# parthjaggi/flow

Measured on AMD Instinct MI355X. Metric: env-steps/sec, higher is better.
Workload: dtype mixed

## Files before the change

flow_amd/csrc/flowsim_pair.h:

```cpp
#pragma once
#include "flowsim_kernels.h"

namespace fs {

typedef float f2 __attribute__((ext_vector_type(2)));
typedef unsigned u2v __attribute__((__vector_size__(8)));

enum : int { DPP_ROW_NEWBCAST0 = 0x150, DPP_ROW_NEWBCAST8 = 0x158 };

__device__ __forceinline__ f2 fma2(f2 a, f2 b, f2 c) { return __builtin_elementwise_fma(a, b, c); }
__device__ __forceinline__ f2 splat(float a) { return f2{a, a}; }

__device__ __forceinline__ f2 pk_mul(f2 a, f2 b) { return a * b; }
__device__ __forceinline__ f2 pk_add(f2 a, f2 b) { return a + b; }
__device__ __forceinline__ f2 pk_sub(f2 a, f2 b) { return a - b; }
__device__ __forceinline__ f2 pk_fma(f2 a, f2 b, f2 c) { return fma2(a, b, c); }
__device__ __forceinline__ f2 pk_fnma(f2 a, f2 b, f2 c) { return fma2(-a, b, c); }
__device__ __forceinline__ float nonneg_else(float x, float y) {
  const unsigned a = __builtin_bit_cast(unsigned, x), b = __builtin_bit_cast(unsigned, y);
  return __builtin_bit_cast(float, min(a, b));
}

template <int ROW>
__device__ __forceinline__ float next_a(float v, bool last, int lane) {
// ... 113 lines not shown
#include "flowsim_pair_step_a_sm.inc"
#undef FS_PAIR_A_NAME
#undef FS_PAIR_A_NZ
#undef FS_PAIR_A_NZ_PARAM
#define FS_PAIR_A_NAME pair_step_asm_a_sm_nz
#define FS_PAIR_A_NZ 1
#define FS_PAIR_A_NZ_PARAM , f2 nz
#include "flowsim_pair_step_a_sm.inc"
#undef FS_PAIR_A_NAME
#undef FS_PAIR_A_NZ
#undef FS_PAIR_A_NZ_PARAM
__device__ __forceinline__ void pair_step_asm_b(f2& V, f2& X, f2& H, f2& DVL, f2& OV, unsigned& crash_bits, float& sq,
                                                const PairConsts& c) {
  asm volatile(
      "v_sub_f32_e32 v118, v112, v113\n"
      "v_sub_f32_e32 v132, v115, v114\n"
      "v_subrev_f32_dpp v119, v112, v113 row_shl:1 row_mask:0xf bank_mask:0xf bound_ctrl:1\n"
      "v_subrev_f32_dpp v134, v112, v113 row_newbcast:0 row_mask:0xf bank_mask:0xf\n"
      "v_sub_f32_dpp v133, v114, v115 row_shl:1 row_mask:0xf bank_mask:0xf bound_ctrl:1\n"
      "v_sub_f32_dpp v135, v114, v115 row_newbcast:0 row_mask:0xf bank_mask:0xf\n"
      "v_cndmask_b32_e64 v119, v119, v134, %[last]\n"
      "v_cndmask_b32_e64 v133, v133, v135, %[last]\n"
      "v_pk_add_f32 v[126:127], v[132:133], %[L2]\n"
      "v_min_u32_e32 v132, v132, v126\n"
      "v_min_u32_e32 v133, v133, v127\n"
      "v_pk_add_f32 v[116:117], v[132:133], %[lenlead] neg_lo:[0,1] neg_hi:[0,1]\n"
      "v_pk_add_f32 v[126:127], v[116:117], %[gap2] neg_lo:[0,1] neg_hi:[0,1]\n"
      "v_min_f32_e32 v126, v126, v127\n"
      "v_alignbit_b32 %[cb], %[cb], v126, 31\n"
      "v_pk_fma_f32 v[124:125], v[112:113], %[vmask], %[tvm]\n"
      "v_pk_mul_f32 v[124:125], v[124:125], v[124:125]\n"
      "v_add_f32_e32 %[sq], v124, v125\n"
      "v_cvt_f64_f32_e32 v[130:131], v112\n"
      "v_cvt_f64_f32_e32 v[132:133], v113\n"
      "v_mul_f64 v[134:135], v[130:131], %[rcms]\n"
      "v_mul_f64 v[136:137], v[132:133], %[rcms]\n"
      "v_fma_f64 v[130:131], -v[134:135], %[ms], v[130:131]\n"
      "v_fma_f64 v[132:133], -v[136:137], %[ms], v[132:133]\n"
      "v_fma_f64 v[134:135], v[130:131], %[rcms], v[134:135]\n"
      "v_fma_f64 v[136:137], v[132:133], %[rcms], v[136:137]\n"
      "v_cvt_f32_f64_e32 v128, v[134:135]\n"
      "v_cvt_f32_f64_e32 v129, v[136:137]\n"
      : "+{v[112:113]}"(V), "+{v[114:115]}"(X), "+{v[116:117]}"(H), "+{v[118:119]}"(DVL), "={v[128:129]}"(OV),
        [cb] "+v"(crash_bits), [sq] "=&v"(sq)
      : [L2] "v"(c.L2), [lenlead] "v"(c.len_lead), [gap2] "v"(c.gap2), [vmask] "v"(c.vmask), [tvm] "v"(c.tvm),
        [ms] "v"(c.ms64), [rcms] "v"(c.rc_ms64), [last] "s"(c.last_mask)
      : "v124", "v125", "v126", "v127", "v130", "v131", "v132", "v133", "v134", "v135", "v136", "v137");
}

struct MixedConsts {
  f2 p0, p1, p2, p5, rc_v0, tsab, rc_ab, one, gap2, vmask, tvm;
  float c1e3;
  double dt, ramp, L, rc_L, rc_ms, len_b, len_next, zero;
  unsigned long long last_mask;
};
__device__ __forceinline__ void mixed_step_asm_a(f2& V32, double& XA, double& XB, double& VA, double& VB, f2& H, f2& DVL,
                                                 f2& OV, const MixedConsts& c) {
  unsigned long long sa, sb;
  asm volatile(
      "v_cmp_nlt_f32_e64 %[sa], |v140|, %[c1e3]\n"
      "v_cmp_nlt_f32_e64 %[sb], |v141|, %[c1e3]\n"
      "v_pk_mul_f32 v[124:125], v[112:113], v[142:143]\n"
      "v_pk_mul_f32 v[126:127], v[124:125], %[rcab]\n"
      "v_pk_fma_f32 v[130:131], v[126:127], %[tsab], v[124:125] neg_lo:[1,0,0] neg_hi:[1,0,0]\n"
      "v_pk_fma_f32 v[126:127], v[130:131], %[rcab], v[126:127]\n"
      "v_cndmask_b32_e64 v120, %[c1e3], v140, %[sa]\n"
      "v_cndmask_b32_e64 v121, %[c1e3], v141, %[sb]\n"
      "v_pk_mul_f32 v[124:125], v[112:113], %[rcv0]\n"
      "v_rcp_f32_e32 v122, v120\n"
      "v_rcp_f32_e32 v123, v121\n"
      "v_pk_fma_f32 v[130:131], v[124:125], %[p0], v[112:113] neg_lo:[1,0,0] neg_hi:[1,0,0]\n"
      "v_pk_fma_f32 v[124:125], v[130:131], %[rcv0], v[124:125]\n"
      "v_pk_mul_f32 v[130:131], v[112:113], %[p1]\n"
      "v_pk_add_f32 v[130:131], v[130:131], v[126:127]\n"
      "v_pk_fma_f32 v[126:127], v[120:121], v[122:123], %[one] neg_lo:[1,0,0] neg_hi:[1,0,0]\n"
      "v_max_f32_e32 v130, 0, v130\n"
      "v_max_f32_e32 v131, 0, v131\n"
      "v_pk_fma_f32 v[122:123], v[126:127], v[122:123], v[122:123]\n"
      "v_pk_add_f32 v[130:131], %[p5], v[130:131]\n"
      "v_pk_mul_f32 v[124:125], v[124:125], v[124:125]\n"
      "v_pk_mul_f32 v[126:127], v[130:131], v[122:123]\n"
      "v_pk_mul_f32 v[124:125], v[124:125], v[124:125]\n"
      "v_pk_fma_f32 v[132:133], v[120:121], v[126:127], v[130:131] neg_lo:[1,0,0] neg_hi:[1,0,0]\n"
      "v_pk_add_f32 v[124:125], %[one], v[124:125] neg_lo:[0,1] neg_hi:[0,1]\n"
      "v_pk_fma_f32 v[126:127], v[132:133], v[122:123], v[126:127]\n"
      "v_pk_fma_f32 v[132:133], v[120:121], v[126:127], v[130:131] neg_lo:[1,0,0] neg_hi:[1,0,0]\n"
      "v_pk_fma_f32 v[126:127], v[132:133], v[122:123], v[126:127]\n"
      "v_pk_mul_f32 v[126:127], v[126:127], v[126:127]\n"
      "v_pk_add_f32 v[124:125], v[124:125], v[126:127] neg_lo:[0,1] neg_hi:[0,1]\n"
      "v_pk_mul_f32 v[124:125], %[p2], v[124:125]\n"
      "v_cvt_f64_f32_e32 v[130:131], v124\n"
      "v_cvt_f64_f32_e32 v[132:133], v125\n"
      "v_mul_f64 v[130:131], v[130:131], %[dt]\n"
      "v_mul_f64 v[132:133], v[132:133], %[dt]\n"
      "v_add_f64 v[130:131], v[118:119], v[130:131]\n"
      "v_add_f64 v[132:133], v[138:139], v[132:133]\n"
      "v_max_f64 v[130:131], v[130:131], %[zero]\n"
      "v_max_f64 v[132:133], v[132:133], %[zero]\n"
      "v_add_f64 v[130:131], v[130:131], -v[118:119]\n"
      "v_add_f64 v[132:133], v[132:133], -v[138:139]\n"
      "v_mul_f64 v[130:131], v[130:131], %[ramp]\n"
      "v_mul_f64 v[132:133], v[132:133], %[ramp]\n"
      "v_add_f64 v[118:119], v[118:119], v[130:131]\n"
      "v_add_f64 v[138:139], v[138:139], v[132:133]\n"
      "v_mul_f64 v[130:131], v[118:119], %[dt]\n"
      "v_mul_f64 v[132:133], v[138:139], %[dt]\n"
      "v_add_f64 v[130:131], v[114:115], v[130:131]\n"
      "v_add_f64 v[132:133], v[116:117], v[132:133]\n"
      "v_add_f64 v[134:135], v[130:131], -%[L]\n"
      "v_add_f64 v[136:137], v[132:133], -%[L]\n"
      "v_cvt_f32_f64_e32 v112, v[118:119]\n"
      "v_cvt_f32_f64_e32 v113, v[138:139]\n"
      "v_cmp_gt_i32_e64 %[sa], 0, v135\n"
      "v_cmp_gt_i32_e64 %[sb], 0, v137\n"
      "v_mul_f64 v[120:121], v[118:119], %[rcms]\n"
      "v_mul_f64 v[122:123], v[138:139], %[rcms]\n"
      "v_cndmask_b32_e64 v114, v134, v130, %[sa]\n"
      "v_cndmask_b32_e64 v115, v135, v131, %[sa]\n"
      "v_cndmask_b32_e64 v116, v136, v132, %[sb]\n"
      "v_cndmask_b32_e64 v117, v137, v133, %[sb]\n"
      "v_cvt_f32_f64_e32 v128, v[120:121]\n"
      "v_cvt_f32_f64_e32 v129, v[122:123]\n"
      : "+{v[112:113]}"(V32), "+{v[114:115]}"(XA), "+{v[116:117]}"(XB), "+{v[118:119]}"(VA), "+{v[138:139]}"(VB),
        "+{v[140:141]}"(H), "+{v[142:143]}"(DVL), "={v[128:129]}"(OV), [sa] "=&s"(sa), [sb] "=&s"(sb)
      : [c1e3] "v"(c.c1e3), [rcab] "v"(c.rc_ab), [tsab] "v"(c.tsab), [rcv0] "v"(c.rc_v0), [p0] "v"(c.p0),
        [p1] "v"(c.p1), [p2] "v"(c.p2), [p5] "v"(c.p5), [one] "v"(c.one), [dt] "v"(c.dt), [ramp] "v"(c.ramp),
        [L] "v"(c.L), [rcms] "v"(c.rc_ms), [zero] "v"(c.zero)
      : "v120", "v121", "v122", "v123", "v124", "v125", "v126", "v127", "v130", "v131", "v132", "v133", "v134",
        "v135", "v136", "v137");
}
struct MixedSumoConsts { double fl0a, fl0b, adta, adtb, ddta, ddtb; };
__device__ __forceinline__ void mixed_step_asm_a_sm(f2& V32, double& XA, double& XB, double& VA, double& VB, f2& H,
                                                    f2& DVL, f2& OV, const MixedConsts& c, const SumoPair& m,
                                                    const MixedSumoConsts& d) {
  unsigned long long sa, sb;
  asm volatile(
      "v_cmp_nlt_f32_e64 %[sa], |v140|, %[c1e3]\n"
      "v_cmp_nlt_f32_e64 %[sb], |v141|, %[c1e3]\n"
      "v_pk_mul_f32 v[124:125], v[112:113], v[142:143]\n"
      "v_pk_mul_f32 v[126:127], v[124:125], %[rcab]\n"
      "v_pk_mul_f32 v[150:151], v[124:125], %[rcts]\n"
      "v_pk_fma_f32 v[130:131], v[126:127], %[tsab], v[124:125] neg_lo:[1,0,0] neg_hi:[1,0,0]\n"
      "v_pk_fma_f32 v[152:153], v[150:151], %[ts], v[124:125] neg_lo:[1,0,0] neg_hi:[1,0,0]\n"
      "v_pk_fma_f32 v[126:127], v[130:131], %[rcab], v[126:127]\n"
      "v_pk_fma_f32 v[150:151], v[152:153], %[rcts], v[150:151]\n"
      "v_cndmask_b32_e64 v120, %[c1e3], v140, %[sa]\n"
      "v_cndmask_b32_e64 v121, %[c1e3], v141, %[sb]\n"
      "v_max_f32_e32 v146, v140, %[c1e3]\n"
      "v_max_f32_e32 v147, v141, %[c1e3]\n"
      "v_pk_mul_f32 v[124:125], v[112:113], %[rcv0]\n"
      "v_rcp_f32_e32 v122, v120\n"
      "v_rcp_f32_e32 v123, v121\n"
      "v_rcp_f32_e32 v148, v146\n"
      "v_rcp_f32_e32 v149, v147\n"
      "v_pk_fma_f32 v[130:131], v[124:125], %[p0], v[112:113] neg_lo:[1,0,0] neg_hi:[1,0,0]\n"
      "v_pk_mul_f32 v[154:155], v[112:113], %[rcsm]\n"
      "v_pk_fma_f32 v[124:125], v[130:131], %[rcv0], v[124:125]\n"
      "v_pk_fma_f32 v[152:153], v[154:155], %[smax], v[112:113] neg_lo:[1,0,0] neg_hi:[1,0,0]\n"
      "v_pk_mul_f32 v[130:131], v[112:113], %[p1]\n"
      "v_pk_fma_f32 v[154:155], v[152:153], %[rcsm], v[154:155]\n"
      "v_pk_add_f32 v[130:131], v[130:131], v[126:127]\n"
      "v_pk_mul_f32 v[152:153], v[112:113], %[tau]\n"
      "v_pk_fma_f32 v[126:127], v[120:121], v[122:123], %[one] neg_lo:[1,0,0] neg_hi:[1,0,0]\n"
      "v_pk_add_f32 v[150:151], v[152:153], v[150:151]\n"
      "v_pk_fma_f32 v[152:153], v[146:147], v[148:149], %[one] neg_lo:[1,0,0] neg_hi:[1,0,0]\n"
      "v_max_f32_e32 v130, 0, v130\n"
      "v_max_f32_e32 v131, 0, v131\n"
      "v_max_f32_e32 v150, 0, v150\n"
      "v_max_f32_e32 v151, 0, v151\n"
      "v_pk_fma_f32 v[122:123], v[126:127], v[122:123], v[122:123]\n"
      "v_pk_fma_f32 v[148:149], v[152:153], v[148:149], v[148:149]\n"
      "v_pk_add_f32 v[130:131], %[p5], v[130:131]\n"
      "v_pk_add_f32 v[150:151], %[mgap], v[150:151]\n"
      "v_pk_mul_f32 v[124:125], v[124:125], v[124:125]\n"
      "v_pk_mul_f32 v[154:155], v[154:155], v[154:155]\n"
      "v_pk_mul_f32 v[126:127], v[130:131], v[122:123]\n"
      "v_pk_mul_f32 v[152:153], v[150:151], v[148:149]\n"
      "v_pk_mul_f32 v[124:125], v[124:125], v[124:125]\n"
      "v_pk_mul_f32 v[154:155], v[154:155], v[154:155]\n"
      "v_pk_fma_f32 v[132:133], v[120:121], v[126:127], v[130:131] neg_lo:[1,0,0] neg_hi:[1,0,0]\n"
      "v_pk_fma_f32 v[134:135], v[146:147], v[152:153], v[150:151] neg_lo:[1,0,0] neg_hi:[1,0,0]\n"
      "v_pk_add_f32 v[124:125], %[one], v[124:125] neg_lo:[0,1] neg_hi:[0,1]\n"
      "v_pk_add_f32 v[154:155], %[one], v[154:155] neg_lo:[0,1] neg_hi:[0,1]\n"
      "v_pk_fma_f32 v[126:127], v[132:133], v[122:123], v[126:127]\n"
      "v_pk_fma_f32 v[152:153], v[134:135], v[148:149], v[152:153]\n"
      "v_pk_fma_f32 v[132:133], v[120:121], v[126:127], v[130:131] neg_lo:[1,0,0] neg_hi:[1,0,0]\n"
      "v_pk_fma_f32 v[134:135], v[146:147], v[152:153], v[150:151] neg_lo:[1,0,0] neg_hi:[1,0,0]\n"
      "v_pk_fma_f32 v[126:127], v[132:133], v[122:123], v[126:127]\n"
      "v_pk_fma_f32 v[152:153], v[134:135], v[148:149], v[152:153]\n"
      "v_pk_mul_f32 v[126:127], v[126:127], v[126:127]\n"
      "v_pk_mul_f32 v[152:153], v[152:153], v[152:153]\n"
      "v_pk_add_f32 v[124:125], v[124:125], v[126:127] neg_lo:[0,1] neg_hi:[0,1]\n"
      "v_pk_add_f32 v[154:155], v[154:155], v[152:153] neg_lo:[0,1] neg_hi:[0,1]\n"
      "v_pk_mul_f32 v[124:125], %[p2], v[124:125]\n"
      "v_pk_mul_f32 v[154:155], %[maxa], v[154:155]\n"
      "v_cvt_f64_f32_e32 v[130:131], v124\n"
      "v_cvt_f64_f32_e32 v[132:133], v125\n"
      "v_cvt_f64_f32_e32 v[134:135], v154\n"
      "v_cvt_f64_f32_e32 v[136:137], v155\n"
      "v_mul_f64 v[130:131], v[130:131], %[dt]\n"
      "v_mul_f64 v[132:133], v[132:133], %[dt]\n"
      "v_mul_f64 v[134:135], v[134:135], %[dt]\n"
      "v_mul_f64 v[136:137], v[136:137], %[dt]\n"
      "v_add_f64 v[130:131], v[118:119], v[130:131]\n"
      "v_add_f64 v[132:133], v[138:139], v[132:133]\n"
      "v_add_f64 v[134:135], v[118:119], v[134:135]\n"
      "v_add_f64 v[136:137], v[138:139], v[136:137]\n"
      "v_max_f64 v[130:131], v[130:131], %[zero]\n"
      "v_max_f64 v[132:133], v[132:133], %[zero]\n"
      "v_max_f64 v[134:135], v[134:135], %[fl0a]\n"
      "v_max_f64 v[136:137], v[136:137], %[fl0b]\n"
      "v_add_f64 v[130:131], v[130:131], -v[118:119]\n"
      "v_add_f64 v[132:133], v[132:133], -v[138:139]\n"
      "v_mul_f64 v[130:131], v[130:131], %[ramp]\n"
      "v_mul_f64 v[132:133], v[132:133], %[ramp]\n"
      "v_add_f64 v[130:131], v[118:119], v[130:131]\n"
      "v_add_f64 v[132:133], v[138:139], v[132:133]\n"
      "v_min_f64 v[130:131], v[130:131], v[134:135]\n"
      "v_min_f64 v[132:133], v[132:133], v[136:137]\n"
      "v_add_f64 v[134:135], v[118:119], %[adta]\n"
      "v_add_f64 v[136:137], v[138:139], %[adtb]\n"
      "v_min_f64 v[130:131], v[130:131], v[134:135]\n"
      "v_min_f64 v[132:133], v[132:133], v[136:137]\n"
      "v_add_f64 v[134:135], v[118:119], -%[ddta]\n"
      "v_add_f64 v[136:137], v[138:139], -%[ddtb]\n"
      "v_max_f64 v[118:119], v[130:131], v[134:135]\n"
      "v_max_f64 v[138:139], v[132:133], v[136:137]\n"
      "v_mul_f64 v[130:131], v[118:119], %[dt]\n"
      "v_mul_f64 v[132:133], v[138:139], %[dt]\n"
      "v_add_f64 v[130:131], v[114:115], v[130:131]\n"
      "v_add_f64 v[132:133], v[116:117], v[132:133]\n"
      "v_add_f64 v[134:135], v[130:131], -%[L]\n"
      "v_add_f64 v[136:137], v[132:133], -%[L]\n"
      "v_cvt_f32_f64_e32 v112, v[118:119]\n"
      "v_cvt_f32_f64_e32 v113, v[138:139]\n"
      "v_cmp_gt_i32_e64 %[sa], 0, v135\n"
      "v_cmp_gt_i32_e64 %[sb], 0, v137\n"
      "v_mul_f64 v[120:121], v[118:119], %[rcms]\n"
      "v_mul_f64 v[122:123], v[138:139], %[rcms]\n"
      "v_cndmask_b32_e64 v114, v134, v130, %[sa]\n"
      "v_cndmask_b32_e64 v115, v135, v131, %[sa]\n"
      "v_cndmask_b32_e64 v116, v136, v132, %[sb]\n"
      "v_cndmask_b32_e64 v117, v137, v133, %[sb]\n"
      "v_cvt_f32_f64_e32 v128, v[120:121]\n"
      "v_cvt_f32_f64_e32 v129, v[122:123]\n"
      : "+{v[112:113]}"(V32), "+{v[114:115]}"(XA), "+{v[116:117]}"(XB), "+{v[118:119]}"(VA), "+{v[138:139]}"(VB),
        "+{v[140:141]}"(H), "+{v[142:143]}"(DVL), "={v[128:129]}"(OV), [sa] "=&s"(sa), [sb] "=&s"(sb)
      : [c1e3] "v"(c.c1e3), [rcab] "v"(c.rc_ab), [tsab] "v"(c.tsab), [rcv0] "v"(c.rc_v0), [p0] "v"(c.p0),
        [p1] "v"(c.p1), [p2] "v"(c.p2), [p5] "v"(c.p5), [one] "v"(c.one), [dt] "v"(c.dt), [ramp] "v"(c.ramp),
        [L] "v"(c.L), [rcms] "v"(c.rc_ms), [zero] "v"(c.zero), [rcts] "v"(m.rc_ts), [ts] "v"(m.ts),
        [rcsm] "v"(m.rc_smax), [smax] "v"(m.smax), [tau] "v"(m.tau), [mgap] "v"(m.min_gap), [maxa] "v"(m.maxa),
        [fl0a] "v"(d.fl0a), [fl0b] "v"(d.fl0b), [adta] "v"(d.adta), [adtb] "v"(d.adtb), [ddta] "v"(d.ddta),
        [ddtb] "v"(d.ddtb)
      : "v120", "v121", "v122", "v123", "v124", "v125", "v126", "v127", "v130", "v131", "v132", "v133", "v134",
        "v135", "v136", "v137", "v146", "v147", "v148", "v149", "v150", "v151", "v152", "v153", "v154", "v155");
}
__device__ __forceinline__ void mixed_step_asm_b(f2& V32, double& XA, double& XB, f2& H, f2& DVL, f2& OX,
                                                 unsigned& crash_bits, float& sq, const MixedConsts& c) {
  unsigned long long sa, sb;
  asm volatile(
      "v_sub_f32_e32 v142, v112, v113\n"
      "v_subrev_f32_dpp v143, v112, v113 row_shl:1 row_mask:0xf bank_mask:0xf bound_ctrl:1\n"
      "v_subrev_f32_dpp v124, v112, v113 row_newbcast:0 row_mask:0xf bank_mask:0xf\n"
      "v_mov_b32_dpp v130, v114 row_shl:1 row_mask:0xf bank_mask:0xf bound_ctrl:1\n"
      "v_mov_b32_dpp v131, v115 row_shl:1 row_mask:0xf bank_mask:0xf bound_ctrl:1\n"
      "v_mov_b32_dpp v132, v114 row_newbcast:0 row_mask:0xf bank_mask:0xf\n"
      "v_mov_b32_dpp v133, v115 row_newbcast:0 row_mask:0xf bank_mask:0xf\n"
      "v_cndmask_b32_e64 v143, v143, v124, %[last]\n"
      "v_cndmask_b32_e64 v130, v130, v132, %[last]\n"
      "v_cndmask_b32_e64 v131, v131, v133, %[last]\n"
      "v_mul_f64 v[120:121], v[114:115], %[rcL]\n"
      "v_mul_f64 v[122:123], v[116:117], %[rcL]\n"
      "v_add_f64 v[134:135], v[116:117], -v[114:115]\n"
      "v_add_f64 v[136:137], v[130:131], -v[116:117]\n"
      "v_cvt_f32_f64_e32 v144, v[120:121]\n"
      "v_cvt_f32_f64_e32 v145, v[122:123]\n"
      "v_add_f64 v[130:131], v[134:135], %[L]\n"
      "v_add_f64 v[132:133], v[136:137], %[L]\n"
      "v_cmp_gt_i32_e64 %[sa], 0, v135\n"
      "v_cmp_gt_i32_e64 %[sb], 0, v137\n"
      "v_pk_fma_f32 v[124:125], v[112:113], %[vmask], %[tvm]\n"
      "v_pk_mul_f32 v[124:125], v[124:125], v[124:125]\n"
      "v_cndmask_b32_e64 v134, v134, v130, %[sa]\n"
      "v_cndmask_b32_e64 v135, v135, v131, %[sa]\n"
      "v_cndmask_b32_e64 v136, v136, v132, %[sb]\n"
      "v_cndmask_b32_e64 v137, v137, v133, %[sb]\n"
      "v_add_f32_e32 %[sq], v124, v125\n"
      "v_add_f64 v[134:135], v[134:135], -%[lenb]\n"
      "v_add_f64 v[136:137], v[136:137], -%[lennext]\n"
      "v_cvt_f32_f64_e32 v140, v[134:135]\n"
      "v_cvt_f32_f64_e32 v141, v[136:137]\n"
      "v_pk_add_f32 v[126:127], v[140:141], %[gap2] neg_lo:[0,1] neg_hi:[0,1]\n"
      "v_min_f32_e32 v126, v126, v127\n"
      "v_alignbit_b32 %[cb], %[cb], v126, 31\n"
      : "+{v[112:113]}"(V32), "+{v[114:115]}"(XA), "+{v[116:117]}"(XB), "+{v[140:141]}"(H), "+{v[142:143]}"(DVL),
        "={v[144:145]}"(OX), [cb] "+v"(crash_bits), [sq] "=&v"(sq), [sa] "=&s"(sa), [sb] "=&s"(sb)
      : [L] "v"(c.L), [rcL] "v"(c.rc_L), [gap2] "v"(c.gap2), [vmask] "v"(c.vmask), [tvm] "v"(c.tvm),
        [lenb] "v"(c.len_b), [lennext] "v"(c.len_next), [last] "s"(c.last_mask)
      : "v120", "v121", "v122", "v123", "v124", "v125", "v126", "v127", "v130", "v131", "v132", "v133", "v134",
        "v135", "v136", "v137");
}

template <typename T, int ROW, bool DELTA4, bool FASTDIV, bool BADCHK, bool SM = false, bool NOISE = false>
__global__ __launch_bounds__(256) void k_rollout_pair(DevView<T> s, int num_steps, float* __restrict__ obs,
                                                      float* __restrict__ rew, uint8_t* __restrict__ done) {
  constexpr bool MIXED = sizeof(T) == 8;
  static_assert(!(NOISE && MIXED), "FS_MIXED has no noise form (its C twin cannot reproduce the hardware's log / cos)");
  constexpr bool ASM = ROW == 16 && DELTA4 && FASTDIV && !BADCHK;
  constexpr int RPW = 64 / ROW;
  constexpr int PERIOD = ROW < 16 ? ROW : 16;
  const int lane = threadIdx.x & 63;
  const int wave = (blockIdx.x * blockDim.x + threadIdx.x) >> 6;
  const int row = lane / ROW;
  const int k = lane % ROW;
  const int r = wave * RPW + row;
  const int N = s.N;
  const int LP = N >> 1;
  const bool rvalid = r < s.R;
  const bool valid = rvalid && k < LP;
  const int rr = rvalid ? r : s.R - 1;
  const int kk = k < LP ? k : LP - 1;
  const bool last = (kk == LP - 1);
  const int iA = 2 * kk, iB = iA + 1;
  const size_t idx = size_t(rr) * N + iA;

  f2 p[6];
#pragma unroll
  for (int q = 0; q < 6; ++q) p[q] = f2{float(s.p[q * N + iA]), float(s.p[q * N + iB])};
  const T lenB = s.length[iB];
  const T len_nextA = next_a<ROW>(T(s.length[iA]), last, lane);
  const T base_len = s.ring_len[rr];
  const T L = base_len + T(4) * s.jlen;
  int tcount = s.time[rr];
  uint32_t nctr = NOISE ? s.noise_ctr[rr] : 0u;
  const f2 sigma = NOISE ? f2{float(s.noise[iA]), float(s.noise[iB])} : f2{0.0f, 0.0f};
  const bool noisyA = NOISE && sigma.x > 0.0f, noisyB = NOISE && sigma.y > 0.0f;
  float gA[4] = {0.0f, 0.0f, 0.0f, 0.0f}, gB[4] = {0.0f, 0.0f, 0.0f, 0.0f};
  if constexpr (NOISE) {
    if ((nctr & 3u) != 0u) {
      gauss4<float>(s.seed_lo, s.seed_hi, s.rep0 + uint32_t(rr), uint32_t(iA), nctr >> 2, gA, s.noise_exact != 0);
      gauss4<float>(s.seed_lo, s.seed_hi, s.rep0 + uint32_t(rr), uint32_t(iB), nctr >> 2, gB, s.noise_exact != 0);
      for (uint32_t q = 0; q < (nctr & 3u); ++q) {
        gA[0] = gA[1]; gA[1] = gA[2]; gA[2] = gA[3];
        gB[0] = gB[1]; gB[1] = gB[2]; gB[2] = gB[3];
      }
    }
  }

  const float dt = float(s.dt), ramp = float(s.ramp);
  const f2 two_sqrt_ab = {2.0f * tsqrt(p[2].x * p[3].x), 2.0f * tsqrt(p[2].y * p[3].y)};
  const f2 rc_v0 = {1.0f / p[0].x, 1.0f / p[0].y}, rc_ab = {1.0f / two_sqrt_ab.x, 1.0f / two_sqrt_ab.y};
  const float Lf = float(L);
  const f2 L2 = splat(Lf), rc_L2 = splat(1.0f / Lf), one = splat(1.0f), dt2 = splat(dt), ramp2 = splat(ramp);
  const f2 gap2 = splat(float(s.crash_gap)), m100 = splat(-100.0f);
  const f2 vmask = splat(valid ? 1.0f : 0.0f), tvm = splat(valid ? -float(s.target_velocity) : 0.0f);
  const double ms64 = double(s.max_speed), rc_ms64 = 1.0 / ms64;
  const double L64 = double(L), rc_L64 = 1.0 / L64, dt64 = double(s.dt), ramp64 = double(s.ramp);

  f2 x, v;
  double xdA = 0, xdB = 0, vdA = 0, vdB = 0;
  if (MIXED) {
    xdA = double(s.pos[idx]); xdB = double(s.pos[idx + 1]);
    vdA = double(s.vel[idx]); vdB = double(s.vel[idx + 1]);
    v = f2{float(vdA), float(vdB)};
    x = f2{0.0f, 0.0f};
  } else {
    x = f2{float(s.pos[idx]), float(s.pos[idx + 1])};
    v = f2{float(s.vel[idx]), float(s.vel[idx + 1])};
  }
  const f2 len_lead = {float(lenB), float(len_nextA)};

  auto headway = [&]() -> f2 {
    if (MIXED) {
      const double xn = next_a<ROW>(xdA, last, lane);
      double dA = xdB - xdA, dB = xn - xdB;
      dA = dA < 0.0 ? dA + L64 : dA;
      dB = dB < 0.0 ? dB + L64 : dB;
      return f2{float(dA - double(lenB)), float(dB - double(len_nextA))};
    } else {
      const f2 xl = {x.y, next_a<ROW>(x.x, last, lane)};
      f2 d = pk_sub(xl, x);
      const f2 dw = pk_add(d, L2);
      d.x = nonneg_else(d.x, dw.x);
      d.y = nonneg_else(d.y, dw.y);
      return pk_sub(d, len_lead);
    }
  };
  f2 h = headway();
  f2 vl = {v.y, next_a<ROW>(v.x, last, lane)};
  f2 dvl = v - vl;
  PairConsts pc;
  pc.p0 = p[0]; pc.p1 = p[1]; pc.p2 = p[2]; pc.p5 = p[5]; pc.rc_v0 = rc_v0; pc.tsab = two_sqrt_ab; pc.rc_ab = rc_ab;
  pc.one = one; pc.dt2 = dt2; pc.ramp2 = ramp2; pc.L2 = L2; pc.rc_L2 = rc_L2; pc.len_lead = len_lead;
  pc.gap2 = gap2; pc.vmask = vmask; pc.tvm = tvm; pc.c1e3 = 1e-3f; pc.ms64 = ms64; pc.rc_ms64 = rc_ms64;
  pc.last_mask = __ballot(last);
  MixedConsts mc;
  mc.p0 = p[0]; mc.p1 = p[1]; mc.p2 = p[2]; mc.p5 = p[5]; mc.rc_v0 = rc_v0; mc.tsab = two_sqrt_ab; mc.rc_ab = rc_ab;
  mc.one = one; mc.gap2 = gap2; mc.vmask = vmask; mc.tvm = tvm; mc.c1e3 = 1e-3f; mc.dt = dt64; mc.ramp = ramp64;
  mc.L = L64; mc.rc_L = rc_L64; mc.rc_ms = rc_ms64; mc.len_b = double(lenB); mc.len_next = double(len_nextA);
  mc.zero = 0.0; mc.last_mask = pc.last_mask;
  SumoPair sc{};
  double floor0A = 0, floor0B = 0, adtA = 0, adtB = 0, ddtA = 0, ddtB = 0;
  if constexpr (SM) {
    const int mA = s.speed_mode[iA], mB = s.speed_mode[iB];
    const float maA = float(s.max_accel[iA]), maB = float(s.max_accel[iB]);
    const float mdA = float(s.max_decel[iA]), mdB = float(s.max_decel[iB]);
    sc.tau = f2{float(s.sumo_tau[iA]), float(s.sumo_tau[iB])};
    sc.min_gap = f2{float(s.sumo_min_gap[iA]), float(s.sumo_min_gap[iB])};
    sc.maxa = f2{maA, maB};
    sc.smax = f2{float(s.sumo_max_speed[iA]), float(s.sumo_max_speed[iB])};
    sc.rc_smax = f2{1.0f / sc.smax.x, 1.0f / sc.smax.y};
    sc.ts = f2{2.0f * tsqrt(maA * mdA), 2.0f * tsqrt(maB * mdB)};
    sc.rc_ts = f2{1.0f / sc.ts.x, 1.0f / sc.ts.y};
    const float BIG = 3.0e38f;
    sc.floor0 = f2{(mA & 1) ? 0.0f : BIG, (mB & 1) ? 0.0f : BIG};
    sc.adt = f2{(mA & 2) ? maA * dt : BIG, (mB & 2) ? maB * dt : BIG};
    sc.ddt = f2{(mA & 4) ? mdA * dt : BIG, (mB & 4) ? mdB * dt : BIG};
    floor0A = double(sc.floor0.x); floor0B = double(sc.floor0.y);
    adtA = (mA & 2) ? double(s.max_accel[iA]) * dt64 : double(BIG);
    adtB = (mB & 2) ? double(s.max_accel[iB]) * dt64 : double(BIG);
    ddtA = (mA & 4) ? double(s.max_decel[iA]) * dt64 : double(BIG);
    ddtB = (mB & 4) ? double(s.max_decel[iB]) * dt64 : double(BIG);
  }
  const MixedSumoConsts msc = {floor0A, floor0B, adtA, adtB, ddtA, ddtB};

  const unsigned rowb = 2u * unsigned(N) * 4u;
  const unsigned off_v = unsigned(rr) * rowb + unsigned(iA) * 4u;
  const unsigned off_x = off_v + unsigned(N) * 4u;
  const size_t step_bytes = size_t(s.R) * rowb;
  const unsigned step_b32 = unsigned(step_bytes);
  char* ob = reinterpret_cast<char*>(obs);
  unsigned crash_bits = 0u, bad_bits = 0u;

  typedef unsigned u4v __attribute__((__vector_size__(16)));
  constexpr bool XPOSE = ASM;
  __shared__ float row_img[XPOSE ? 4 : 1][XPOSE ? RPW * 64 : 1];
  float* const my_img = row_img[XPOSE ? (threadIdx.x >> 6) & 3 : 0] + (XPOSE ? row * 2 * N : 0);
  const unsigned off_16 = unsigned(rr) * rowb + unsigned(kk) * 16u;
  u4v piece = {0u, 0u, 0u, 0u};
  auto transpose_in = [&](f2 ov, f2 ox) {
    *reinterpret_cast<f2*>(my_img + 2 * kk) = ov;
    *reinterpret_cast<f2*>(my_img + N + 2 * kk) = ox;
    __builtin_amdgcn_fence(__ATOMIC_RELEASE, "wavefront");
    __builtin_amdgcn_wave_barrier();
    __builtin_amdgcn_fence(__ATOMIC_ACQUIRE, "wavefront");
    piece = *reinterpret_cast<const u4v*>(my_img + 4 * kk);
  };

  auto noise_term = [&]() -> f2 {
    f2 nz = {-0.0f, -0.0f};
    if constexpr (NOISE) {
      const bool fresh = (nctr & 3u) == 0u;
      if (__ballot(fresh) != 0ull) {
        if (fresh) {
          gauss4<float>(s.seed_lo, s.seed_hi, s.rep0 + uint32_t(rr), uint32_t(iA), nctr >> 2, gA, s.noise_exact != 0);
          gauss4<float>(s.seed_lo, s.seed_hi, s.rep0 + uint32_t(rr), uint32_t(iB), nctr >> 2, gB, s.noise_exact != 0);
        }
      }
      const float tA = sigma.x * gA[0], tB = sigma.y * gB[0];
      nz.x = noisyA ? tA : -0.0f;
      nz.y = noisyB ? tB : -0.0f;
      gA[0] = gA[1]; gA[1] = gA[2]; gA[2] = gA[3];
      gB[0] = gB[1]; gB[1] = gB[2]; gB[2] = gB[3];
      nctr += 1u;
    }
    return nz;
  };

  auto one_step = [&](int slot, __amdgpu_buffer_rsrc_t rs, float& sq_out) {
    if constexpr (ASM) {
      f2 ov, ox;
      const unsigned so = unsigned(slot) * step_b32;
      if constexpr (MIXED) {
        if constexpr (SM) mixed_step_asm_a_sm(v, xdA, xdB, vdA, vdB, h, dvl, ov, mc, sc, msc);
        else mixed_step_asm_a(v, xdA, xdB, vdA, vdB, h, dvl, ov, mc);
        if (slot > 0) __builtin_amdgcn_raw_buffer_store_b128(piece, rs, off_16, so - step_b32, 0);
        mixed_step_asm_b(v, xdA, xdB, h, dvl, ox, crash_bits, sq_out, mc);
        transpose_in(ov, ox);
      } else {
#if defined(FS_DIAG_NOSTORE)
        pair_step_asm_a(v, x, h, dvl, ox, pc);
        pair_step_asm_b(v, x, h, dvl, ov, crash_bits, sq_out, pc);
        asm volatile("" :: "v"(ov), "v"(ox), "s"(so));
#elif defined(FS_DIAG_NOXPOSE)
        pair_step_asm_a(v, x, h, dvl, ox, pc);
        __builtin_amdgcn_raw_buffer_store_b64(__builtin_bit_cast(u2v, ox), rs, off_x, so, 0);
        pair_step_asm_b(v, x, h, dvl, ov, crash_bits, sq_out, pc);
        __builtin_amdgcn_raw_buffer_store_b64(__builtin_bit_cast(u2v, ov), rs, off_v, so, 0);
#else
        if constexpr (NOISE) {
          const f2 nz = noise_term();
          if constexpr (SM) pair_step_asm_a_sm_nz(v, x, h, dvl, ox, pc, sc, nz);
          else pair_step_asm_a_nz(v, x, h, dvl, ox, pc, nz);
        } else {
          if constexpr (SM) pair_step_asm_a_sm(v, x, h, dvl, ox, pc, sc);
          else pair_step_asm_a(v, x, h, dvl, ox, pc);
        }
        if (slot > 0) __builtin_amdgcn_raw_buffer_store_b128(piece, rs, off_16, so - step_b32, 0);
        pair_step_asm_b(v, x, h, dvl, ov, crash_bits, sq_out, pc);
        transpose_in(ov, ox);
#endif
      }
      return;
    }
    f2 acc = idm_pair<DELTA4, FASTDIV>(v, vl, h, p, two_sqrt_ab, rc_ab, rc_v0, one);
    if constexpr (NOISE) acc = pk_add(acc, noise_term());
    f2 acc_s = {0.0f, 0.0f};
    if constexpr (SM) acc_s = sumo_acc_pair<FASTDIV>(v, vl, h, sc, one);
    f2 ox;
    if (MIXED) {
      const double aA = double(acc.x), aB = double(acc.y);
      const double nA = tmax(vdA + aA * dt64, 0.0), nB = tmax(vdB + aB * dt64, 0.0);
      double cA = vdA + (nA - vdA) * ramp64, cB = vdB + (nB - vdB) * ramp64;
      if constexpr (SM) {
        const double sA = tmax(vdA + double(acc_s.x) * dt64, floor0A), sB = tmax(vdB + double(acc_s.y) * dt64, floor0B);
        cA = tmin(cA, sA); cB = tmin(cB, sB);
        cA = tmin(cA, vdA + adtA); cB = tmin(cB, vdB + adtB);
        cA = tmax(cA, vdA - ddtA); cB = tmax(cB, vdB - ddtB);
      }
      vdA = cA;
      vdB = cB;
      const double xA = xdA + vdA * dt64, xB = xdB + vdB * dt64;
      xdA = xA >= L64 ? xA - L64 : xA;
      xdB = xB >= L64 ? xB - L64 : xB;
      v = f2{float(vdA), float(vdB)};
      ox = f2{float(xdA * rc_L64), float(xdB * rc_L64)};
    } else {
      f2 nv = pk_add(v, pk_mul(acc, dt2));
      nv.x = tmax(nv.x, 0.0f);
      nv.y = tmax(nv.y, 0.0f);
// ... 119 lines not shown
```

Before: 13.62 billion.

## Split mixed-precision step into fast path and rare ring-wrap slow path

Ring-road position wrapping, per-follower wrap offsets and headway clamping leave the common mixed-precision step. A cheap bit-pattern check (max3 on exponent words plus a threshold) decides per wave whether any lane needs a wrap or clamp, and only then runs a separate slow-path asm block. Wrap offsets are carried across steps in registers, and the headway clamp is applied once up front and then inside the slow path. This removes compares and selects from every step but adds a wave-wide branch and relies on the threshold check being conservative enough to stay correct.

```diff
diff --git a/flow_amd/csrc/flowsim_pair.h b/flow_amd/csrc/flowsim_pair.h
--- a/flow_amd/csrc/flowsim_pair.h
+++ b/flow_amd/csrc/flowsim_pair.h
@@ -189,28 +189,24 @@
   f2 p0, p1, p2, p5, rc_v0, tsab, rc_ab, one, gap2, vmask, tvm;
   float c1e3;
   double dt, ramp, L, rc_L, rc_ms, len_b, len_next, zero;
+  unsigned L_lo, L_hi, thr;
   unsigned long long last_mask;
 };
 __device__ __forceinline__ void mixed_step_asm_a(f2& V32, double& XA, double& XB, double& VA, double& VB, f2& H, f2& DVL,
                                                  f2& OV, const MixedConsts& c) {
-  unsigned long long sa, sb;
   asm volatile(
-      "v_cmp_nlt_f32_e64 %[sa], |v140|, %[c1e3]\n"
-      "v_cmp_nlt_f32_e64 %[sb], |v141|, %[c1e3]\n"
       "v_pk_mul_f32 v[124:125], v[112:113], v[142:143]\n"
       "v_pk_mul_f32 v[126:127], v[124:125], %[rcab]\n"
       "v_pk_fma_f32 v[130:131], v[126:127], %[tsab], v[124:125] neg_lo:[1,0,0] neg_hi:[1,0,0]\n"
       "v_pk_fma_f32 v[126:127], v[130:131], %[rcab], v[126:127]\n"
-      "v_cndmask_b32_e64 v120, %[c1e3], v140, %[sa]\n"
-      "v_cndmask_b32_e64 v121, %[c1e3], v141, %[sb]\n"
       "v_pk_mul_f32 v[124:125], v[112:113], %[rcv0]\n"
-      "v_rcp_f32_e32 v122, v120\n"
-      "v_rcp_f32_e32 v123, v121\n"
+      "v_rcp_f32_e32 v122, v140\n"
+      "v_rcp_f32_e32 v123, v141\n"
       "v_pk_fma_f32 v[130:131], v[124:125], %[p0], v[112:113] neg_lo:[1,0,0] neg_hi:[1,0,0]\n"
       "v_pk_fma_f32 v[124:125], v[130:131], %[rcv0], v[124:125]\n"
       "v_pk_mul_f32 v[130:131], v[112:113], %[p1]\n"
       "v_pk_add_f32 v[130:131], v[130:131], v[126:127]\n"
-      "v_pk_fma_f32 v[126:127], v[120:121], v[122:123], %[one] neg_lo:[1,0,0] neg_hi:[1,0,0]\n"
+      "v_pk_fma_f32 v[126:127], v[140:141], v[122:123], %[one] neg_lo:[1,0,0] neg_hi:[1,0,0]\n"
       "v_max_f32_e32 v130, 0, v130\n"
       "v_max_f32_e32 v131, 0, v131\n"
       "v_pk_fma_f32 v[122:123], v[126:127], v[122:123], v[122:123]\n"
@@ -218,10 +214,10 @@
       "v_pk_mul_f32 v[124:125], v[124:125], v[124:125]\n"
       "v_pk_mul_f32 v[126:127], v[130:131], v[122:123]\n"
       "v_pk_mul_f32 v[124:125], v[124:125], v[124:125]\n"
-      "v_pk_fma_f32 v[132:133], v[120:121], v[126:127], v[130:131] neg_lo:[1,0,0] neg_hi:[1,0,0]\n"
+      "v_pk_fma_f32 v[132:133], v[140:141], v[126:127], v[130:131] neg_lo:[1,0,0] neg_hi:[1,0,0]\n"
       "v_pk_add_f32 v[124:125], %[one], v[124:125] neg_lo:[0,1] neg_hi:[0,1]\n"
       "v_pk_fma_f32 v[126:127], v[132:133], v[122:123], v[126:127]\n"
-      "v_pk_fma_f32 v[132:133], v[120:121], v[126:127], v[130:131] neg_lo:[1,0,0] neg_hi:[1,0,0]\n"
+      "v_pk_fma_f32 v[132:133], v[140:141], v[126:127], v[130:131] neg_lo:[1,0,0] neg_hi:[1,0,0]\n"
       "v_pk_fma_f32 v[126:127], v[132:133], v[122:123], v[126:127]\n"
       "v_pk_mul_f32 v[126:127], v[126:127], v[126:127]\n"
       "v_pk_add_f32 v[124:125], v[124:125], v[126:127] neg_lo:[0,1] neg_hi:[0,1]\n"
@@ -240,40 +236,27 @@
       "v_mul_f64 v[132:133], v[132:133], %[ramp]\n"
       "v_add_f64 v[118:119], v[118:119], v[130:131]\n"
       "v_add_f64 v[138:139], v[138:139], v[132:133]\n"
+      "v_cvt_f32_f64_e32 v112, v[118:119]\n"
+      "v_cvt_f32_f64_e32 v113, v[138:139]\n"
       "v_mul_f64 v[130:131], v[118:119], %[dt]\n"
       "v_mul_f64 v[132:133], v[138:139], %[dt]\n"
-      "v_add_f64 v[130:131], v[114:115], v[130:131]\n"
-      "v_add_f64 v[132:133], v[116:117], v[132:133]\n"
-      "v_add_f64 v[134:135], v[130:131], -%[L]\n"
-      "v_add_f64 v[136:137], v[132:133], -%[L]\n"
-      "v_cvt_f32_f64_e32 v112, v[118:119]\n"
-      "v_cvt_f32_f64_e32 v113, v[138:139]\n"
-      "v_cmp_gt_i32_e64 %[sa], 0, v135\n"
-      "v_cmp_gt_i32_e64 %[sb], 0, v137\n"
+      "v_add_f64 v[114:115], v[114:115], v[130:131]\n"
+      "v_add_f64 v[116:117], v[116:117], v[132:133]\n"
       "v_mul_f64 v[120:121], v[118:119], %[rcms]\n"
       "v_mul_f64 v[122:123], v[138:139], %[rcms]\n"
-      "v_cndmask_b32_e64 v114, v134, v130, %[sa]\n"
-      "v_cndmask_b32_e64 v115, v135, v131, %[sa]\n"
-      "v_cndmask_b32_e64 v116, v136, v132, %[sb]\n"
-      "v_cndmask_b32_e64 v117, v137, v133, %[sb]\n"
       "v_cvt_f32_f64_e32 v128, v[120:121]\n"
       "v_cvt_f32_f64_e32 v129, v[122:123]\n"
       : "+{v[112:113]}"(V32), "+{v[114:115]}"(XA), "+{v[116:117]}"(XB), "+{v[118:119]}"(VA), "+{v[138:139]}"(VB),
-        "+{v[140:141]}"(H), "+{v[142:143]}"(DVL), "={v[128:129]}"(OV), [sa] "=&s"(sa), [sb] "=&s"(sb)
-      : [c1e3] "v"(c.c1e3), [rcab] "v"(c.rc_ab), [tsab] "v"(c.tsab), [rcv0] "v"(c.rc_v0), [p0] "v"(c.p0),
-        [p1] "v"(c.p1), [p2] "v"(c.p2), [p5] "v"(c.p5), [one] "v"(c.one), [dt] "v"(c.dt), [ramp] "v"(c.ramp),
-        [L] "v"(c.L), [rcms] "v"(c.rc_ms), [zero] "v"(c.zero)
-      : "v120", "v121", "v122", "v123", "v124", "v125", "v126", "v127", "v130", "v131", "v132", "v133", "v134",
-        "v135", "v136", "v137");
+        "+{v[140:141]}"(H), "+{v[142:143]}"(DVL), "={v[128:129]}"(OV)
+      : [rcab] "v"(c.rc_ab), [tsab] "v"(c.tsab), [rcv0] "v"(c.rc_v0), [p0] "v"(c.p0), [p1] "v"(c.p1), [p2] "v"(c.p2),
+        [p5] "v"(c.p5), [one] "v"(c.one), [dt] "v"(c.dt), [ramp] "v"(c.ramp), [rcms] "v"(c.rc_ms), [zero] "v"(c.zero)
+      : "v120", "v121", "v122", "v123", "v124", "v125", "v126", "v127", "v130", "v131", "v132", "v133");
 }
 struct MixedSumoConsts { double fl0a, fl0b, adta, adtb, ddta, ddtb; };
 __device__ __forceinline__ void mixed_step_asm_a_sm(f2& V32, double& XA, double& XB, double& VA, double& VB, f2& H,
                                                     f2& DVL, f2& OV, const MixedConsts& c, const SumoPair& m,
                                                     const MixedSumoConsts& d) {
-  unsigned long long sa, sb;
   asm volatile(
-      "v_cmp_nlt_f32_e64 %[sa], |v140|, %[c1e3]\n"
-      "v_cmp_nlt_f32_e64 %[sb], |v141|, %[c1e3]\n"
       "v_pk_mul_f32 v[124:125], v[112:113], v[142:143]\n"
       "v_pk_mul_f32 v[126:127], v[124:125], %[rcab]\n"
       "v_pk_mul_f32 v[150:151], v[124:125], %[rcts]\n"
@@ -281,13 +264,11 @@
       "v_pk_fma_f32 v[152:153], v[150:151], %[ts], v[124:125] neg_lo:[1,0,0] neg_hi:[1,0,0]\n"
       "v_pk_fma_f32 v[126:127], v[130:131], %[rcab], v[126:127]\n"
       "v_pk_fma_f32 v[150:151], v[152:153], %[rcts], v[150:151]\n"
-      "v_cndmask_b32_e64 v120, %[c1e3], v140, %[sa]\n"
-      "v_cndmask_b32_e64 v121, %[c1e3], v141, %[sb]\n"
       "v_max_f32_e32 v146, v140, %[c1e3]\n"
       "v_max_f32_e32 v147, v141, %[c1e3]\n"
       "v_pk_mul_f32 v[124:125], v[112:113], %[rcv0]\n"
-      "v_rcp_f32_e32 v122, v120\n"
-      "v_rcp_f32_e32 v123, v121\n"
+      "v_rcp_f32_e32 v122, v140\n"
+      "v_rcp_f32_e32 v123, v141\n"
       "v_rcp_f32_e32 v148, v146\n"
       "v_rcp_f32_e32 v149, v147\n"
       "v_pk_fma_f32 v[130:131], v[124:125], %[p0], v[112:113] neg_lo:[1,0,0] neg_hi:[1,0,0]\n"
@@ -298,7 +279,7 @@
       "v_pk_fma_f32 v[154:155], v[152:153], %[rcsm], v[154:155]\n"
       "v_pk_add_f32 v[130:131], v[130:131], v[126:127]\n"
       "v_pk_mul_f32 v[152:153], v[112:113], %[tau]\n"
-      "v_pk_fma_f32 v[126:127], v[120:121], v[122:123], %[one] neg_lo:[1,0,0] neg_hi:[1,0,0]\n"
+      "v_pk_fma_f32 v[126:127], v[140:141], v[122:123], %[one] neg_lo:[1,0,0] neg_hi:[1,0,0]\n"
       "v_pk_add_f32 v[150:151], v[152:153], v[150:151]\n"
       "v_pk_fma_f32 v[152:153], v[146:147], v[148:149], %[one] neg_lo:[1,0,0] neg_hi:[1,0,0]\n"
       "v_max_f32_e32 v130, 0, v130\n"
@@ -315,13 +296,13 @@
       "v_pk_mul_f32 v[152:153], v[150:151], v[148:149]\n"
       "v_pk_mul_f32 v[124:125], v[124:125], v[124:125]\n"
       "v_pk_mul_f32 v[154:155], v[154:155], v[154:155]\n"
-      "v_pk_fma_f32 v[132:133], v[120:121], v[126:127], v[130:131] neg_lo:[1,0,0] neg_hi:[1,0,0]\n"
+      "v_pk_fma_f32 v[132:133], v[140:141], v[126:127], v[130:131] neg_lo:[1,0,0] neg_hi:[1,0,0]\n"
       "v_pk_fma_f32 v[134:135], v[146:147], v[152:153], v[150:151] neg_lo:[1,0,0] neg_hi:[1,0,0]\n"
       "v_pk_add_f32 v[124:125], %[one], v[124:125] neg_lo:[0,1] neg_hi:[0,1]\n"
       "v_pk_add_f32 v[154:155], %[one], v[154:155] neg_lo:[0,1] neg_hi:[0,1]\n"
       "v_pk_fma_f32 v[126:127], v[132:133], v[122:123], v[126:127]\n"
       "v_pk_fma_f32 v[152:153], v[134:135], v[148:149], v[152:153]\n"
-      "v_pk_fma_f32 v[132:133], v[120:121], v[126:127], v[130:131] neg_lo:[1,0,0] neg_hi:[1,0,0]\n"
+      "v_pk_fma_f32 v[132:133], v[140:141], v[126:127], v[130:131] neg_lo:[1,0,0] neg_hi:[1,0,0]\n"
       "v_pk_fma_f32 v[134:135], v[146:147], v[152:153], v[150:151] neg_lo:[1,0,0] neg_hi:[1,0,0]\n"
       "v_pk_fma_f32 v[126:127], v[132:133], v[122:123], v[126:127]\n"
       "v_pk_fma_f32 v[152:153], v[134:135], v[148:149], v[152:153]\n"
@@ -363,38 +344,30 @@
       "v_add_f64 v[136:137], v[138:139], -%[ddtb]\n"
       "v_max_f64 v[118:119], v[130:131], v[134:135]\n"
       "v_max_f64 v[138:139], v[132:133], v[136:137]\n"
+      "v_cvt_f32_f64_e32 v112, v[118:119]\n"
+      "v_cvt_f32_f64_e32 v113, v[138:139]\n"
       "v_mul_f64 v[130:131], v[118:119], %[dt]\n"
       "v_mul_f64 v[132:133], v[138:139], %[dt]\n"
-      "v_add_f64 v[130:131], v[114:115], v[130:131]\n"
-      "v_add_f64 v[132:133], v[116:117], v[132:133]\n"
-      "v_add_f64 v[134:135], v[130:131], -%[L]\n"
-      "v_add_f64 v[136:137], v[132:133], -%[L]\n"
-      "v_cvt_f32_f64_e32 v112, v[118:119]\n"
-      "v_cvt_f32_f64_e32 v113, v[138:139]\n"
-      "v_cmp_gt_i32_e64 %[sa], 0, v135\n"
-      "v_cmp_gt_i32_e64 %[sb], 0, v137\n"
+      "v_add_f64 v[114:115], v[114:115], v[130:131]\n"
+      "v_add_f64 v[116:117], v[116:117], v[132:133]\n"
       "v_mul_f64 v[120:121], v[118:119], %[rcms]\n"
       "v_mul_f64 v[122:123], v[138:139], %[rcms]\n"
-      "v_cndmask_b32_e64 v114, v134, v130, %[sa]\n"
-      "v_cndmask_b32_e64 v115, v135, v131, %[sa]\n"
-      "v_cndmask_b32_e64 v116, v136, v132, %[sb]\n"
-      "v_cndmask_b32_e64 v117, v137, v133, %[sb]\n"
       "v_cvt_f32_f64_e32 v128, v[120:121]\n"
       "v_cvt_f32_f64_e32 v129, v[122:123]\n"
       : "+{v[112:113]}"(V32), "+{v[114:115]}"(XA), "+{v[116:117]}"(XB), "+{v[118:119]}"(VA), "+{v[138:139]}"(VB),
-        "+{v[140:141]}"(H), "+{v[142:143]}"(DVL), "={v[128:129]}"(OV), [sa] "=&s"(sa), [sb] "=&s"(sb)
+        "+{v[140:141]}"(H), "+{v[142:143]}"(DVL), "={v[128:129]}"(OV)
       : [c1e3] "v"(c.c1e3), [rcab] "v"(c.rc_ab), [tsab] "v"(c.tsab), [rcv0] "v"(c.rc_v0), [p0] "v"(c.p0),
         [p1] "v"(c.p1), [p2] "v"(c.p2), [p5] "v"(c.p5), [one] "v"(c.one), [dt] "v"(c.dt), [ramp] "v"(c.ramp),
-        [L] "v"(c.L), [rcms] "v"(c.rc_ms), [zero] "v"(c.zero), [rcts] "v"(m.rc_ts), [ts] "v"(m.ts),
+        [rcms] "v"(c.rc_ms), [zero] "v"(c.zero), [rcts] "v"(m.rc_ts), [ts] "v"(m.ts),
         [rcsm] "v"(m.rc_smax), [smax] "v"(m.smax), [tau] "v"(m.tau), [mgap] "v"(m.min_gap), [maxa] "v"(m.maxa),
         [fl0a] "v"(d.fl0a), [fl0b] "v"(d.fl0b), [adta] "v"(d.adta), [adtb] "v"(d.adtb), [ddta] "v"(d.ddta),
         [ddtb] "v"(d.ddtb)
       : "v120", "v121", "v122", "v123", "v124", "v125", "v126", "v127", "v130", "v131", "v132", "v133", "v134",
         "v135", "v136", "v137", "v146", "v147", "v148", "v149", "v150", "v151", "v152", "v153", "v154", "v155");
 }
-__device__ __forceinline__ void mixed_step_asm_b(f2& V32, double& XA, double& XB, f2& H, f2& DVL, f2& OX,
-                                                 unsigned& crash_bits, float& sq, const MixedConsts& c) {
-  unsigned long long sa, sb;
+__device__ __forceinline__ void mixed_step_asm_b(f2& V32, double& XA, double& XB, f2& H, f2& DVL, f2& OX, const double& WA,
+                                                 const double& WB, float& ct, float& sq, unsigned long long& need,
+                                                 const MixedConsts& c) {
   asm volatile(
       "v_sub_f32_e32 v142, v112, v113\n"
       "v_subrev_f32_dpp v143, v112, v113 row_shl:1 row_mask:0xf bank_mask:0xf bound_ctrl:1\n"
@@ -403,39 +376,89 @@
       "v_mov_b32_dpp v131, v115 row_shl:1 row_mask:0xf bank_mask:0xf bound_ctrl:1\n"
       "v_mov_b32_dpp v132, v114 row_newbcast:0 row_mask:0xf bank_mask:0xf\n"
       "v_mov_b32_dpp v133, v115 row_newbcast:0 row_mask:0xf bank_mask:0xf\n"
-      "v_cndmask_b32_e64 v143, v143, v124, %[last]\n"
+      "v_add_f64 v[134:135], v[116:117], -v[114:115]\n"
       "v_cndmask_b32_e64 v130, v130, v132, %[last]\n"
       "v_cndmask_b32_e64 v131, v131, v133, %[last]\n"
+      "v_add_f64 v[134:135], v[134:135], %[wa]\n"
+      "v_add_f64 v[136:137], v[130:131], -v[116:117]\n"
+      "v_cndmask_b32_e64 v143, v143, v124, %[last]\n"
+      "v_add_f64 v[120:121], v[134:135], -%[lenb]\n"
+      "v_add_f64 v[136:137], v[136:137], %[wb]\n"
+      "v_max3_u32 v126, v115, v117, v135\n"
+      "v_add_f64 v[122:123], v[136:137], -%[lennext]\n"
+      "v_cvt_f32_f64_e32 v140, v[120:121]\n"
+      "v_cvt_f32_f64_e32 v141, v[122:123]\n"
+      "v_min_f32_e32 v127, v140, v141\n"
+      "v_sub_u32_e32 v125, v127, %[c1e3]\n"
+      "v_max3_u32 v126, v126, v137, v125\n"
+      "v_cmp_le_u32_e64 %[need], %[thr], v126\n"
+      "v_mul_f64 v[120:121], v[114:115], %[rcL]\n"
+      "v_mul_f64 v[122:123], v[116:117], %[rcL]\n"
+      "v_pk_fma_f32 v[124:125], v[112:113], %[vmask], %[tvm]\n"
+      "v_cvt_f32_f64_e32 v144, v[120:121]\n"
+      "v_cvt_f32_f64_e32 v145, v[122:123]\n"
+      "v_pk_mul_f32 v[124:125], v[124:125], v[124:125]\n"
+      "v_sub_f32_e32 %[ct], v127, %[gap]\n"
+      "v_add_f32_e32 %[sq], v124, v125\n"
+      : "+{v[112:113]}"(V32), "+{v[114:115]}"(XA), "+{v[116:117]}"(XB), "+{v[140:141]}"(H), "+{v[142:143]}"(DVL),
+        "=&{v[144:145]}"(OX), [ct] "=&v"(ct), [sq] "=&v"(sq), [need] "=&s"(need)
+      : [wa] "{v[156:157]}"(WA), [wb] "{v[158:159]}"(WB), [rcL] "v"(c.rc_L), [gap] "v"(c.gap2.x), [vmask] "v"(c.vmask), [tvm] "v"(c.tvm),
+        [lenb] "v"(c.len_b), [lennext] "v"(c.len_next), [c1e3] "v"(c.c1e3), [thr] "v"(c.thr), [last] "s"(c.last_mask)
+      : "v120", "v121", "v122", "v123", "v124", "v125", "v126", "v127", "v130", "v131", "v132", "v133", "v134", "v135",
+        "v136", "v137");
+}
+__device__ __forceinline__ void mixed_step_asm_slow(double& XA, double& XB, f2& H, f2& OX, double& WA, double& WB, float& ct,
+                                                    const MixedConsts& c) {
+  unsigned long long sa, sb;
+  asm volatile(
+      "v_add_f64 v[134:135], v[114:115], -%[L]\n"
+      "v_add_f64 v[136:137], v[116:117], -%[L]\n"
+      "v_cmp_gt_i32_e64 %[sa], 0, v135\n"
+      "v_cmp_gt_i32_e64 %[sb], 0, v137\n"
+      "s_nop 0\n"
+      "v_cndmask_b32_e64 v114, v134, v114, %[sa]\n"
+      "v_cndmask_b32_e64 v115, v135, v115, %[sa]\n"
+      "v_cndmask_b32_e64 v116, v136, v116, %[sb]\n"
+      "v_cndmask_b32_e64 v117, v137, v117, %[sb]\n"
       "v_mul_f64 v[120:121], v[114:115], %[rcL]\n"
       "v_mul_f64 v[122:123], v[116:117], %[rcL]\n"
       "v_add_f64 v[134:135], v[116:117], -v[114:115]\n"
-      "v_add_f64 v[136:137], v[130:131], -v[116:117]\n"
       "v_cvt_f32_f64_e32 v144, v[120:121]\n"
       "v_cvt_f32_f64_e32 v145, v[122:123]\n"
-      "v_add_f64 v[130:131], v[134:135], %[L]\n"
+      "v_add_f64 v[126:127], v[134:135], %[L]\n"
+      "v_mov_b32_dpp v130, v114 row_shl:1 row_mask:0xf bank_mask:0xf bound_ctrl:1\n"
+      "v_mov_b32_dpp v131, v115 row_shl:1 row_mask:0xf bank_mask:0xf bound_ctrl:1\n"
+      "v_mov_b32_dpp v132, v114 row_newbcast:0 row_mask:0xf bank_mask:0xf\n"
+      "v_mov_b32_dpp v133, v115 row_newbcast:0 row_mask:0xf bank_mask:0xf\n"
+      "v_cmp_gt_i32_e64 %[sa], 0, v135\n"
+      "v_cndmask_b32_e64 v130, v130, v132, %[last]\n"
+      "v_cndmask_b32_e64 v131, v131, v133, %[last]\n"
+      "v_add_f64 v[136:137], v[130:131], -v[116:117]\n"
+      "v_cndmask_b32_e64 v134, v134, v126, %[sa]\n"
+      "v_cndmask_b32_e64 v135, v135, v127, %[sa]\n"
+      "v_cndmask_b32_e64 v156, 0, %[Llo], %[sa]\n"
+      "v_cndmask_b32_e64 v157, 0, %[Lhi], %[sa]\n"
       "v_add_f64 v[132:133], v[136:137], %[L]\n"
-      "v_cmp_gt_i32_e64 %[sa], 0, v135\n"
       "v_cmp_gt_i32_e64 %[sb], 0, v137\n"
-      "v_pk_fma_f32 v[124:125], v[112:113], %[vmask], %[tvm]\n"
-      "v_pk_mul_f32 v[124:125], v[124:125], v[124:125]\n"
-      "v_cndmask_b32_e64 v134, v134, v130, %[sa]\n"
-      "v_cndmask_b32_e64 v135, v135, v131, %[sa]\n"
+      "v_add_f64 v[134:135], v[134:135], -%[lenb]\n"
+      "v_cvt_f32_f64_e32 v140, v[134:135]\n"
       "v_cndmask_b32_e64 v136, v136, v132, %[sb]\n"
       "v_cndmask_b32_e64 v137, v137, v133, %[sb]\n"
-      "v_add_f32_e32 %[sq], v124, v125\n"
-      "v_add_f64 v[134:135], v[134:135], -%[lenb]\n"
+      "v_cndmask_b32_e64 v158, 0, %[Llo], %[sb]\n"
+      "v_cndmask_b32_e64 v159, 0, %[Lhi], %[sb]\n"
       "v_add_f64 v[136:137], v[136:137], -%[lennext]\n"
-      "v_cvt_f32_f64_e32 v140, v[134:135]\n"
       "v_cvt_f32_f64_e32 v141, v[136:137]\n"
       "v_pk_add_f32 v[126:127], v[140:141], %[gap2] neg_lo:[0,1] neg_hi:[0,1]\n"
-      "v_min_f32_e32 v126, v126, v127\n"
-      "v_alignbit_b32 %[cb], %[cb], v126, 31\n"
-      : "+{v[112:113]}"(V32), "+{v[114:115]}"(XA), "+{v[116:117]}"(XB), "+{v[140:141]}"(H), "+{v[142:143]}"(DVL),
-        "={v[144:145]}"(OX), [cb] "+v"(crash_bits), [sq] "=&v"(sq), [sa] "=&s"(sa), [sb] "=&s"(sb)
-      : [L] "v"(c.L), [rcL] "v"(c.rc_L), [gap2] "v"(c.gap2), [vmask] "v"(c.vmask), [tvm] "v"(c.tvm),
-        [lenb] "v"(c.len_b), [lennext] "v"(c.len_next), [last] "s"(c.last_mask)
-      : "v120", "v121", "v122", "v123", "v124", "v125", "v126", "v127", "v130", "v131", "v132", "v133", "v134",
-        "v135", "v136", "v137");
+      "v_cmp_nlt_f32_e64 %[sa], |v140|, %[c1e3]\n"
+      "v_cmp_nlt_f32_e64 %[sb], |v141|, %[c1e3]\n"
+      "v_min_f32_e32 %[ct], v126, v127\n"
+      "v_cndmask_b32_e64 v140, %[c1e3], v140, %[sa]\n"
+      "v_cndmask_b32_e64 v141, %[c1e3], v141, %[sb]\n"
+      : "+{v[114:115]}"(XA), "+{v[116:117]}"(XB), "+{v[140:141]}"(H), "+{v[144:145]}"(OX), "+{v[156:157]}"(WA),
+        "+{v[158:159]}"(WB), [ct] "+v"(ct), [sa] "=&s"(sa), [sb] "=&s"(sb)
+      : [L] "v"(c.L), [Llo] "v"(c.L_lo), [Lhi] "v"(c.L_hi), [rcL] "v"(c.rc_L), [gap2] "v"(c.gap2), [lenb] "v"(c.len_b),
+        [lennext] "v"(c.len_next), [c1e3] "v"(c.c1e3), [last] "s"(c.last_mask)
+      : "v120", "v121", "v122", "v123", "v126", "v127", "v130", "v131", "v132", "v133", "v134", "v135", "v136", "v137");
 }
 
 template <typename T, int ROW, bool DELTA4, bool FASTDIV, bool BADCHK, bool SM = false, bool NOISE = false>
@@ -536,6 +559,20 @@
   mc.one = one; mc.gap2 = gap2; mc.vmask = vmask; mc.tvm = tvm; mc.c1e3 = 1e-3f; mc.dt = dt64; mc.ramp = ramp64;
   mc.L = L64; mc.rc_L = rc_L64; mc.rc_ms = rc_ms64; mc.len_b = double(lenB); mc.len_next = double(len_nextA);
   mc.zero = 0.0; mc.last_mask = pc.last_mask;
+  {
+    const unsigned long long Lb = __builtin_bit_cast(unsigned long long, L64);
+    mc.L_lo = unsigned(Lb); mc.L_hi = unsigned(Lb >> 32);
+    mc.thr = mc.L_hi < 0x457CED91u ? mc.L_hi : 0x457CED91u;
+  }
+  double wA = 0.0, wB = 0.0;
+  if constexpr (ASM && MIXED) {
+    asm volatile("" : "+v"(mc.dt), "+v"(mc.ramp), "+v"(mc.one), "+v"(mc.zero), "+v"(mc.rc_ms), "+v"(mc.c1e3), "+v"(mc.gap2));
+    const double xn = next_a<ROW>(xdA, last, lane);
+    wA = xdB - xdA < 0.0 ? L64 : 0.0;
+    wB = xn - xdB < 0.0 ? L64 : 0.0;
+    h.x = tabs(h.x) < 1e-3f ? 1e-3f : h.x;
+    h.y = tabs(h.y) < 1e-3f ? 1e-3f : h.y;
+  }
   SumoPair sc{};
   double floor0A = 0, floor0B = 0, adtA = 0, adtB = 0, ddtA = 0, ddtB = 0;
   if constexpr (SM) {
@@ -612,7 +649,16 @@
         if constexpr (SM) mixed_step_asm_a_sm(v, xdA, xdB, vdA, vdB, h, dvl, ov, mc, sc, msc);
         else mixed_step_asm_a(v, xdA, xdB, vdA, vdB, h, dvl, ov, mc);
         if (slot > 0) __builtin_amdgcn_raw_buffer_store_b128(piece, rs, off_16, so - step_b32, 0);
-        mixed_step_asm_b(v, xdA, xdB, h, dvl, ox, crash_bits, sq_out, mc);
+        float ct;
+        unsigned long long need;
+        mixed_step_asm_b(v, xdA, xdB, h, dvl, ox, wA, wB, ct, sq_out, need, mc);
+#if defined(FS_DIAG_ALWAYS_SLOW)
+        need = ~0ull;
+#elif defined(FS_DIAG_NEVER_SLOW)
+        need = 0ull;
+#endif
+        if (__builtin_expect(need != 0ull, 0)) mixed_step_asm_slow(xdA, xdB, h, ox, wA, wB, ct, mc);
+        crash_bits = __builtin_amdgcn_alignbit(crash_bits, __builtin_bit_cast(unsigned, ct), 31);
         transpose_in(ov, ox);
       } else {
 #if defined(FS_DIAG_NOSTORE)
```

New measurement: 14.02 billion (median of 6 runs). 2.9% higher.
